# fferflo/semantic-meshes

Hardware: AMD Instinct MI355X
Metric: views/sec fused (1080p, 19 classes, 1M-tri mesh) (higher is better)
Workload: dtype f32; 1 GPU; cfg2: 1000000-triangle grid mesh, 11763 views/GPU at 1920x1080, 19 classes, probs resident in HBM; views_per_call=8, group_pipeline=True, repeats=1, allreduce=none, exchange=allreduce, nranks=1, allreduce_bytes=0, exchange_parts=1, held_views=0

## Files before the change

semantic_meshes_amd/_lib.py:

```python
import ctypes
import os
import threading

_HERE = os.path.dirname(os.path.abspath(__file__))
LIB_PATH = os.environ.get("SMESH_LIB_PATH") or os.path.join(_HERE, "csrc", "libsmesh_hip.so")

OK, ERR_INVALID, ERR_RUNTIME, ERR_NODEVICE = 0, 1, 2, 3
MEM_HOST, MEM_DEVICE = 0, 1
IDX_U32, IDX_I32, IDX_U64, IDX_I64 = 0, 1, 2, 3
AGG_KINDS = {"Sum": 0, "Summax": 1, "Mul": 2}
PROF_FUSE_SCATTER, PROF_FUSE_HIST, PROF_RASTER, PROF_FINALIZE, PROF_EXCHANGE = 0, 1, 2, 3, 4

c_void_p, c_int, c_u64, c_u32, c_float = ctypes.c_void_p, ctypes.c_int, ctypes.c_uint64, ctypes.c_uint32, ctypes.c_float
P = ctypes.POINTER


class CameraPOD(ctypes.Structure):
    _fields_ = [
        ("rotation", ctypes.c_float * 9),
        ("translation", ctypes.c_float * 3),
        ("focal", ctypes.c_double * 2),
        ("principal", ctypes.c_double * 2),
        ("width", ctypes.c_uint64),
        ("height", ctypes.c_uint64),
# ... 111 lines not shown
EVAL_SIGNATURES = {
    "smesh_confusion_create": (c_int, [c_u32, c_int, P(c_void_p)]),
    "smesh_confusion_destroy": (c_int, [c_void_p]),
    "smesh_confusion_reset": (c_int, [c_void_p]),
    "smesh_confusion_get": (c_int, [c_void_p, c_void_p, P(c_u64)]),
    "smesh_confusion_add_counts": (c_int, [c_void_p, c_void_p, c_u64]),
    "smesh_confusion_add_labels": (c_int, [c_void_p, c_void_p, c_int, c_void_p, c_int, c_int, c_u64]),
    "smesh_aggregator_labels": (c_int, [c_void_p, c_float, c_void_p, c_int]),
    "smesh_confusion_add_image": (c_int, [c_void_p, c_void_p, c_int, P(ctypes.c_int64), c_int, c_void_p, c_u64, c_int,
                                          c_void_p, c_int, P(ctypes.c_int64), c_int, c_u64, c_u64]),
    "smesh_confusion_add_view": (c_int, [c_void_p, c_void_p, P(CameraPOD), c_void_p, c_u64, c_void_p, c_int, P(ctypes.c_int64), c_int]),
    "smesh_confusion_add_views": (c_int, [c_void_p, c_void_p, P(CameraPOD), c_u64, c_void_p, c_u64, P(c_void_p), c_int,
                                          P(ctypes.c_int64), c_int]),
}

_lib = None
_lock = threading.Lock()


def _elf_dynamic_strings(path):
    import struct
    with open(path, "rb") as f:
        data = f.read()
    try:
        if data[:6] != b"\x7fELF\x02\x01":
            raise ValueError("not a little-endian ELF64 file")
        phoff, = struct.unpack_from("<Q", data, 0x20)
        phentsize, phnum = struct.unpack_from("<HH", data, 0x36)
        loads, dyn = [], None
        for k in range(phnum):
# ... 81 lines not shown
    if os.path.exists(rccl):
        os.environ.setdefault("SMESH_RCCL_LIB", rccl)


def lib():
    global _lib
    if _lib is None:
        with _lock:
            if _lib is None:
                if not os.path.exists(LIB_PATH):
                    raise RuntimeError(
                        "semantic_meshes_amd: %s not found -- build it with `make -C semantic_meshes_amd/csrc` "
                        "(or `python -c 'import __graft_entry__ as g; g.build()'`). There is no CPU fallback." % LIB_PATH)
                _preload_hip_runtime()
                L = ctypes.CDLL(LIB_PATH)
                for name, (res, args) in list(SIGNATURES.items()) + list(EXT_SIGNATURES.items()) + list(VERTEX_SIGNATURES.items()) + list(EVAL_SIGNATURES.items()):
                    fn = getattr(L, name)
                    fn.restype = res
                    fn.argtypes = args
                _lib = L
    return _lib


def check(status):
    if status == OK:
        return
    msg = lib().smesh_last_error().decode(errors="replace")
    if status == ERR_INVALID:
        raise ValueError(msg)
    raise RuntimeError(msg)

# ... 29 lines not shown
```

semantic_meshes_amd/csrc/common.hpp:

```cpp
#pragma once

#include <hip/hip_runtime.h>

#include <cstdint>
#include <cstdio>
#include <cstdlib>
#include <functional>
#include <mutex>
#include <string>
#include <vector>

#include "../../include/smesh.h"

namespace smesh {

int fail(int code, const std::string& msg);
int fail_hip(hipError_t e, const char* what, const char* file, int line);

#define SMESH_HIP(expr)                                                         \
  do {                                                                          \
    hipError_t _e = (expr);                                                     \
    if (_e != hipSuccess) return ::smesh::fail_hip(_e, #expr, __FILE__, __LINE__); \
  } while (0)

// ... 41 lines not shown
  bool counted = false;
  ProfScope(DeviceCtx* c, int s, hipStream_t stream = nullptr);
  ~ProfScope();
};

void prof_note(DeviceCtx* ctx, int slot, uint64_t launches, uint64_t views);

hipError_t dev_malloc(void** out, size_t bytes);
hipError_t dev_free(void* p, bool foreign = false);
uint64_t dev_cached_bytes(int device);
void dev_trim(int device);
void dev_cache_stats(uint64_t* live_blocks, uint64_t* cached_blocks, uint64_t* cached_bytes);

bool opt_group_pipeline();
bool opt_confusion_wave_aggregate();

constexpr uint32_t kConfusionLdsMaxC = 180;

struct Scratch {
  void* ptr = nullptr;
  size_t bytes = 0;
  int reserve(size_t need);
  void release();
};

inline uint64_t div_up(uint64_t a, uint64_t b) { return (a + b - 1) / b; }

inline int env_int(const char* name, int def) {
  const char* e = getenv(name);
  return e ? atoi(e) : def;
// ... 109 lines not shown
```

semantic_meshes_amd/csrc/context.cpp:

```cpp
#include "common.hpp"
#include "labels_scratch.hpp"

#include <algorithm>
#include <atomic>

#include <cstdlib>
#include <cstring>
#include <map>
#include <memory>
#include <unordered_map>
#include <vector>

namespace smesh {

static thread_local std::string g_err;

int fail(int code, const std::string& msg) {
  g_err = msg;
  return code;
}

int fail_hip(hipError_t e, const char* what, const char* file, int line) {
  char buf[512];
  snprintf(buf, sizeof buf, "HIP error %d (%s) at %s:%d: %s", (int)e, hipGetErrorString(e), file, line, what);
  g_err = buf;
  (void)hipGetLastError();
  return (e == hipErrorNoDevice || e == hipErrorInvalidDevice) ? SMESH_ERR_NODEVICE : SMESH_ERR_RUNTIME;
}

static std::atomic<int> g_confusion_wave_aggregate{1};
bool opt_confusion_wave_aggregate() { return g_confusion_wave_aggregate.load() != 0; }

static std::atomic<int> g_group_pipeline{-1};
bool opt_group_pipeline() {
  int v = g_group_pipeline.load();
  if (v < 0) {
    const char* e = getenv("SMESH_GROUP_PIPELINE");
    v = e ? (atoi(e) != 0 ? 1 : 0) : 1;
    g_group_pipeline.store(v);
  }
  return v != 0;
}

static std::mutex g_ctx_mu;
static std::vector<std::unique_ptr<DeviceCtx>> g_ctx;

// ... 233 lines not shown

using namespace smesh;

void smesh_last_fuse_instance(int* slot, int* views);

extern "C" {

const char* smesh_backend(void) { return "hip-gfx950"; }

const char* smesh_last_error(void) { return g_err.c_str(); }

int smesh_set_option(const char* name, int64_t value) {
  if (!name) return fail(SMESH_ERR_INVALID, "option name is NULL");
  if (!strcmp(name, "group_pipeline")) { g_group_pipeline.store(value != 0 ? 1 : 0); return SMESH_OK; }
  if (!strcmp(name, "confusion_wave_aggregate")) { g_confusion_wave_aggregate.store(value != 0 ? 1 : 0); return SMESH_OK; }
  return fail(SMESH_ERR_INVALID, std::string("unknown option: ") + name);
}
int smesh_get_option(const char* name, int64_t* value) {
  if (!name || !value) return fail(SMESH_ERR_INVALID, "NULL argument");
  if (!strcmp(name, "group_pipeline")) { *value = opt_group_pipeline() ? 1 : 0; return SMESH_OK; }
  if (!strcmp(name, "labels_lds_max_classes")) { *value = (int64_t)kLabelsLdsMaxC; return SMESH_OK; }
  if (!strcmp(name, "confusion_lds_max_classes")) { *value = (int64_t)kConfusionLdsMaxC; return SMESH_OK; }
  if (!strcmp(name, "confusion_wave_aggregate")) { *value = opt_confusion_wave_aggregate() ? 1 : 0; return SMESH_OK; }
  const bool want_slot = !strcmp(name, "last_fuse_slot");
  if (want_slot || !strcmp(name, "last_fuse_views")) {
    int slot, views;
    smesh_last_fuse_instance(&slot, &views);
    *value = want_slot ? slot : views;
    return SMESH_OK;
  }
  return fail(SMESH_ERR_INVALID, std::string("unknown option: ") + name);
}

int smesh_device_count(int* count) {
  if (!count) return fail(SMESH_ERR_INVALID, "count is NULL");
  int n = 0;
  if (hipGetDeviceCount(&n) != hipSuccess) {
    (void)hipGetLastError();
// ... 259 lines not shown
```

semantic_meshes_amd/csrc/raster.hip:

```cpp
#include "common.hpp"

#include <algorithm>
#include <cmath>
#include <cstdlib>
#include <cstring>
#include <new>
#include <string>
#include <utility>
#include <vector>

#pragma clang fp contract(off)

using namespace smesh;

struct smesh_aggregator;
int smesh_aggregator_add_device_contig(smesh_aggregator* a, const uint32_t* d_idx, const float* d_probs,
                                       const float* d_w, uint64_t W, uint64_t H);
bool smesh_aggregator_can_fuse_triangles(smesh_aggregator* a, uint64_t F);
bool smesh_aggregator_can_fuse_pair(smesh_aggregator* a);
int smesh_aggregator_max_fused_views(smesh_aggregator* a);
bool smesh_aggregator_takes_strided_probs(smesh_aggregator* a, int64_t ps0, int64_t ps1, int nviews);
int smesh_aggregator_dense_probs(smesh_aggregator* a, const float* d_probs, const int64_t ps[3], uint64_t W, uint64_t H, const float** out);
bool smesh_aggregator_fuses_small_views_by_mask(smesh_aggregator* a);
int smesh_aggregator_fuse_triangles(smesh_aggregator* a, uint64_t F, const uint32_t* prim_id, uint32_t big_capacity,
// ... 43 lines not shown
  s.u = 0.0; s.v = 0.0; s.iz = 0.0;
  const bool fin = isfinite(xc) && isfinite(yc) && isfinite(zc);
  if (zc > kNear && fin) {
    const double zd = (double)zc;
    const double u = cam.fx * ((double)xc / zd) + cam.cx;
    const double v = cam.fy * ((double)yc / zd) + cam.cy;
    if (isfinite(u) && isfinite(v)) {
      s.u = u; s.v = v; s.iz = 1.0 / zd;
    }
  } else if (fin) {
    s.iz = kBehind;
  }
  return s;
}

__device__ __forceinline__ void project_vertex(const float* __restrict__ verts, uint64_t V, const CameraArgs& cam,
                                               ScreenVertex* __restrict__ sv, uint32_t* __restrict__ big_count, const uint64_t i) {
  if (i == 0) { big_count[0] = 0u; big_count[1] = 0u; big_count[2] = 0u; big_count[3] = 0u; big_count[4] = 0u; big_count[5] = 0u; }
  if (i >= V) return;
  sv[i] = project_point(cam, verts[3 * i + 0], verts[3 * i + 1], verts[3 * i + 2]);
}

__global__ void k_project_vertices(const float* __restrict__ verts, uint64_t V, CameraArgs cam,
                                   ScreenVertex* __restrict__ sv, uint32_t* __restrict__ big_count) {
  project_vertex(verts, V, cam, sv, big_count, (uint64_t)blockIdx.x * blockDim.x + threadIdx.x);
}

constexpr int kMaxGroup = 8;
struct ProjectGroup {
  const float* verts;
  uint64_t V;
  CameraArgs cam[kMaxGroup];
  ScreenVertex* sv[kMaxGroup];
  uint32_t* big_count[kMaxGroup];
  uint32_t n;
};
__global__ void k_project_vertices_group(ProjectGroup g) {
  const uint64_t i = (uint64_t)blockIdx.x * blockDim.x + threadIdx.x;
  if (i == 0)
    for (uint32_t v = 0; v < g.n; v++)
      for (int k = 0; k < 6; k++) g.big_count[v][k] = 0u;
  if (i >= g.V) return;
  const float X = g.verts[3 * i + 0], Y = g.verts[3 * i + 1], Z = g.verts[3 * i + 2];
  for (uint32_t v = 0; v < g.n; v++) g.sv[v][i] = project_point(g.cam[v], X, Y, Z);
}

struct EdgeEq {
  double A, B, C;
};

__device__ __forceinline__ EdgeEq make_edge(double ax, double ay, double bx, double by) {
  EdgeEq e;
  const bool sw = (bx < ax) || (bx == ax && by < ay);
  const double lx = sw ? bx : ax, ly = sw ? by : ay;
  e.A = ay - by;
  e.B = bx - ax;
// ... 108 lines not shown
  uint64_t F, V;
  uint32_t W, H;
  uint32_t* big_queue;
  uint32_t* huge_queue;
  uint32_t* big_count;
  uint32_t big_capacity;
  TriFrag* frags;
  uint8_t* kinds;
  FragQueues q;
  uint32_t tpw;
  uint32_t groups;
  uint32_t* med_queue;
  uint32_t balance;
  uint32_t wg_push;
  uint32_t spread;
  uint32_t idx_optional;
};

__device__ __forceinline__ uint64_t key_index(uint32_t x, uint32_t y, uint32_t H) { return (uint64_t)x * H + y; }

__device__ __forceinline__ bool load_tri(const RasterArgs& a, uint64_t f, Tri& t, const int32_t i0, const int32_t i1, const int32_t i2);
__device__ __forceinline__ bool load_tri(const RasterArgs& a, uint64_t f, Tri& t) {
  return load_tri(a, f, t, a.faces[3 * f + 0], a.faces[3 * f + 1], a.faces[3 * f + 2]);
}
__device__ __forceinline__ bool load_tri(const RasterArgs& a, uint64_t f, Tri& t, const int32_t i0, const int32_t i1, const int32_t i2) {
  if ((uint64_t)max((uint32_t)i0, max((uint32_t)i1, (uint32_t)i2)) >= a.V) return false;
  if (a.tex_res && a.tex_res[f] == 0) return false;
  const ScreenVertex va = a.sv[i0], vb = a.sv[i1], vc = a.sv[i2];
  return setup_tri(va, vb, vc, a.W, a.H, t);
}
// ... 570 lines not shown
  for (uint32_t i = wave; i < turns; i += nwaves) {
    const int tri = lane / kLanes;
    const uint32_t e = i * (uint32_t)kTris + (uint32_t)tri;
    uint64_t fs = a.F;
    if (tri < kTris && e < nl) fs = a.med_queue[a.big_capacity - 1u - e];
    int32_t s0 = 0, s1 = 0, s2 = 0;
    if (fs < a.F) { s0 = a.faces[3 * fs + 0]; s1 = a.faces[3 * fs + 1]; s2 = a.faces[3 * fs + 2]; }
    raster_frag_64<TEX ? 6 : 2>(a, fs, s0, s1, s2, i & (kQSub - 1), lane % kLanes, true);
  }
}
template <bool TEX>
__global__ __launch_bounds__(256) void k_raster_medium(RasterArgs a) {
  raster_medium_wave<TEX>(a, (blockIdx.x * blockDim.x + threadIdx.x) >> 6, (gridDim.x * blockDim.x) >> 6);
}

template <bool LOOP, int MODE>
__device__ __forceinline__ void raster_frag_wave(const RasterArgs& a, const uint64_t wave_id) {
  const int lane = threadIdx.x & 63;
  if constexpr ((MODE & 2) != 0) {
    const int tri = lane / kSpread;
    uint64_t fs = wave_id * (uint64_t)kSpreadTris + (uint64_t)tri;
    if (tri >= kSpreadTris || fs >= a.F) fs = a.F;
    int32_t s0 = 0, s1 = 0, s2 = 0;
    if (fs < a.F) { s0 = a.faces[3 * fs + 0]; s1 = a.faces[3 * fs + 1]; s2 = a.faces[3 * fs + 2]; }
    raster_frag_64<MODE>(a, fs, s0, s1, s2, (uint32_t)wave_id & (kQSub - 1), lane % kSpread);
    return;
  } else {
  const uint32_t G = LOOP ? a.groups : 1u;
  uint64_t f = lane < (int)a.tpw ? wave_id * G * a.tpw + lane : a.F;
  int32_t n0 = 0, n1 = 0, n2 = 0;
  if (f < a.F) { n0 = a.faces[3 * f + 0]; n1 = a.faces[3 * f + 1]; n2 = a.faces[3 * f + 2]; }
  for (uint32_t g = 0; g < G; g++) {
    const int32_t i0 = n0, i1 = n1, i2 = n2;
    const uint64_t fn = f + 64u;
    if (g + 1 < G && fn < a.F) { n0 = a.faces[3 * fn + 0]; n1 = a.faces[3 * fn + 1]; n2 = a.faces[3 * fn + 2]; }
    raster_frag_64<MODE>(a, f, i0, i1, i2, (uint32_t)(wave_id * G + g) & (kQSub - 1));
    f = fn < a.F ? fn : a.F;
  }
  }
}

__device__ __forceinline__ uint32_t xcd_block(const uint32_t xcd, const uint32_t s, const uint32_t run) {
  const uint32_t q = s / run;
  return (q * 8u + xcd) * run + (s - q * run);
}
inline uint32_t xcd_slots(uint32_t nblocks, uint32_t run) { return (uint32_t)div_up(nblocks, 8u * run) * run; }

template <int MODE>
__global__ __launch_bounds__(256) __attribute__((amdgpu_waves_per_eu((MODE & 3) ? 4 : 5, 5))) void k_raster_frag(RasterArgs a, uint32_t nblocks, uint32_t chunk) {
  const uint32_t tb = chunk ? xcd_block(blockIdx.x & 7u, blockIdx.x >> 3, chunk) : blockIdx.x;
  if (tb >= nblocks) return;
  raster_frag_wave<false, MODE>(a, ((uint64_t)tb * blockDim.x + threadIdx.x) >> 6);
// ... 281 lines not shown

struct ImagePair {
  uint32_t* idx;
  float* depth;
  uint64_t pixels;
  bool idx_out, depth_out;
};

struct smesh_renderer {
  DeviceCtx* ctx = nullptr;
  uint64_t V = 0, F = 0, num_primitives = 0;
  float* verts = nullptr;
  int32_t* faces = nullptr;
  struct Bounds { bool valid = false; double lo[3] = {0, 0, 0}, hi[3] = {0, 0, 0}, max_edge = 0, mean_edge = 0; } bounds;
  uint32_t* prim_id = nullptr;
  struct ViewScratch {
    ScreenVertex* sv = nullptr;
    uint32_t* huge_queue = nullptr;
    uint32_t* med_queue = nullptr;
    unsigned long long* keys = nullptr;
    uint64_t keys_pixels = 0;
    FragQueues fq;
    uint64_t fq_tiles = 0;
  } vs[kSlots];
  bool texels = false;
  uint32_t* tex_res = nullptr;
  uint32_t* tex_first = nullptr;
  std::vector<int32_t> h_faces;
  std::vector<uint32_t> h_res, h_first;
  struct Side {
    uint32_t* big_queue = nullptr;
    uint32_t* big_count = nullptr;
    TriFrag* frags = nullptr;
    uint8_t* kinds = nullptr;
// ... 184 lines not shown
                       const smesh_camera_t* cam = nullptr) {
  RasterArgs a;
  a.faces = r->faces; a.verts = r->verts; a.sv = vs.sv; a.tex_res = r->texels ? r->tex_res : nullptr; a.tex_first = r->tex_first;
  a.prim_id = r->prim_id;
  a.keys = vs.keys; a.F = r->F; a.V = r->V; a.W = (uint32_t)W; a.H = (uint32_t)H;
  a.big_queue = r->side[side].big_queue; a.big_count = r->side[side].big_count; a.big_capacity = r->big_capacity;
  a.huge_queue = vs.huge_queue;
  a.med_queue = vs.med_queue;
  {
    static const int knob = env_int("SMESH_RASTER_BALANCE", -1);
    a.balance = (vs.med_queue && (knob >= 0 ? knob != 0 : (cam && depth_spread(r, cam) > 6.0))) ? (nviews > 1 ? 1u : 2u) : 0u;
  }
  a.frags = r->side[side].frags;
  a.kinds = r->side[side].kinds;
  a.q = FragQueues();
  a.idx_optional = 0u;
  a.tpw = 64;
  const bool fine = r->F >= 32768u;
  const uint64_t min_waves = fine ? 1024u : 2048u;
  const uint64_t launch_views = fine ? (uint64_t)std::max(1, nviews) : 1u;
  while (a.tpw > 1 && launch_views * r->F / a.tpw < min_waves) a.tpw >>= 1;
  a.groups = 1;
  a.spread = 0u;
  {
    static const int knob = env_int("SMESH_RASTER_WG_PUSH", -1);
    a.wg_push = knob >= 0 ? (uint32_t)(knob != 0) : (cam && typical_edge_pixels(r, cam) >= 5.0 ? 1u : 0u);
  }
  if (want_spread(r, cam, nviews)) { a.spread = (uint32_t)kSpread; a.tpw = (uint32_t)kSpreadTris; }
  return a;
}

uint32_t frag_groups(uint64_t F, int views, uint32_t tpw) {
  static const int knob = env_int("SMESH_RASTER_GROUPS", 0);
  if (tpw != 64u) return 1u;
  if (knob >= 1) return (uint32_t)knob;
  return (F >= 4000000u && (uint64_t)views * div_up(F, 256u) >= 20480u) ? 4u : 1u;
}

int render_into(smesh_renderer* r, const smesh_camera_t* cam, uint32_t* d_idx, float* d_depth, hipStream_t st = nullptr,
                int side = 0, int idx_optional = 0) {
  DeviceCtx* ctx = r->ctx;
  r->last_render_side = side;
  if (!st) {
    st = ctx->stream;
    SMESH_TRY(main_after_raster(r));
    r->main_pending = true;
  }
  const uint64_t W = cam->width, H = cam->height, N = W * H;
  smesh_renderer::ViewScratch& vs = r->vs[0];
  SMESH_TRY(ensure_keys(vs, W, H, st));
  ProfScope prof(ctx, SMESH_PROF_RASTER, st);
  const CameraArgs ca = camera_args(cam);
  RasterArgs a = raster_args(r, vs, side, W, H, 1, cam);
  a.cam = ca;
  if (r->V) {
    hipLaunchKernelGGL(k_project_vertices, dim3((uint32_t)div_up(r->V, 256)), dim3(256), 0, st, r->verts, r->V, ca, vs.sv,
                       r->side[side].big_count);
    SMESH_HIP(hipGetLastError());
  } else {
    SMESH_HIP(hipMemsetAsync(r->side[side].big_count, 0, 32, st));
  }
  if (r->F) {
    a.idx_optional = (idx_optional && plane_optional_allowed(r)) ? (uint32_t)idx_optional : 0u;
    const uint32_t big_grid = (uint32_t)std::min<uint64_t>(r->F, (uint64_t)ctx->num_cus);
    int qs = SMESH_OK;
    if (raster_path() == RasterPath::Frag && ensure_queues(r, vs, W, H, st, &qs)) {
      a.q = vs.fq;
      {
        const uint32_t nblocks = (uint32_t)div_up(div_up(r->F, a.tpw), 4);
        const uint32_t chunk = nblocks >= 64u ? kRasterXcdRun : 0u;
        const dim3 grid(chunk ? 8u * xcd_slots(nblocks, chunk) : nblocks);
        switch (raster_mode(a)) {
// ... 20 lines not shown
    }
    SMESH_TRY(qs);
    hipLaunchKernelGGL(k_raster_small, dim3((uint32_t)div_up(r->F, 256)), dim3(256), 0, st, a);
    SMESH_HIP(hipGetLastError());
    hipLaunchKernelGGL(k_raster_big, dim3(big_grid), dim3(256), 0, st, a, 0u);
    SMESH_HIP(hipGetLastError());
  }
  hipLaunchKernelGGL(k_resolve, dim3((uint32_t)div_up(N, 256)), dim3(256), 0, st, vs.keys, d_idx, d_depth, (uint32_t)W, (uint32_t)H);
  SMESH_HIP(hipGetLastError());
  SMESH_HIP(hipMemsetAsync(r->side[side].big_count + 1, 0xFF, 4, st));
  return SMESH_OK;
}

hipError_t alloc_side(smesh_renderer* r, int i);

hipError_t alloc_scratch(smesh_renderer* r, int i) {
  smesh_renderer::ViewScratch& vs = r->vs[i];
  hipError_t e = hipSuccess;
  if (!vs.sv) e = dev_malloc(reinterpret_cast<void**>(&vs.sv), std::max<uint64_t>(r->V * sizeof(ScreenVertex), 16));
  if (e == hipSuccess && !vs.huge_queue) e = dev_malloc(reinterpret_cast<void**>(&vs.huge_queue), (size_t)r->big_capacity * 4);
  if (e == hipSuccess && !vs.med_queue) e = dev_malloc(reinterpret_cast<void**>(&vs.med_queue), (size_t)r->big_capacity * 4);
  return e;
}

bool queues_fit_group(uint64_t W, uint64_t H) {
  if (raster_path() != RasterPath::Frag) return false;
  if (frag_cap_forced()) return true;
  const uint64_t ntiles = div_up(W, kQW) * div_up(H, kQH);
  const uint64_t cap = 16ull * kQPixels / kQSub;
  return ntiles * kQSub * cap * 10 <= (2ull << 30);
}

int prepare_group_slots(smesh_renderer* r, const smesh_camera_t* cams, int n, hipStream_t st, int base) {
  for (int v = 0; v < n; v++) {
    const uint64_t W = cams[v].width, H = cams[v].height, N = W * H;
    SMESH_HIP(alloc_side(r, base + v));
// ... 52 lines not shown
  rg.n = (uint32_t)n;
  {
    int votes = 0;
    for (int v = 0; v < n; v++) votes += want_spread(r, &cams[v], n) ? 1 : 0;
    if (2 * votes >= n && votes > 0)
      for (int v = 0; v < n; v++) { rg.view[v].spread = (uint32_t)kSpread; rg.view[v].tpw = (uint32_t)kSpreadTris; }
    int push_votes = 0;
    for (int v = 0; v < n; v++) push_votes += rg.view[v].wg_push ? 1 : 0;
    for (int v = 0; v < n; v++) rg.view[v].wg_push = 2 * push_votes >= n && push_votes > 0 ? 1u : 0u;
    int balance_votes = 0;
    for (int v = 0; v < n; v++) balance_votes += rg.view[v].balance ? 1 : 0;
    for (int v = 0; v < n; v++) rg.view[v].balance = 2 * balance_votes >= n && balance_votes > 0 ? (n > 1 ? 1u : 2u) : 0u;
  }
  for (int v = 0; v < n; v++) rg.view[v].groups = frag_groups(r->F, n, rg.view[0].tpw);
  rg.blocks_per_view = (uint32_t)div_up(div_up(r->F, rg.view[0].tpw * rg.view[0].groups), 4);
  ProfScope prof(ctx, SMESH_PROF_RASTER, st);
  hipLaunchKernelGGL(k_project_vertices_group, dim3((uint32_t)div_up(r->V, 256)), dim3(256), 0, st, pg);
  SMESH_HIP(hipGetLastError());
  {
    rg.chunk = rg.blocks_per_view >= 64u ? kRasterXcdRun : 0u;
    const dim3 grid(rg.chunk ? 8u * xcd_slots(rg.blocks_per_view, rg.chunk) * (uint32_t)n : (uint32_t)n * rg.blocks_per_view);
    switch (raster_mode(rg.view[0])) {
      case 7:  hipLaunchKernelGGL(k_raster_frag_group<7>, grid, dim3(256), 0, st, rg); break;
      case 5:  hipLaunchKernelGGL(k_raster_frag_group<5>, grid, dim3(256), 0, st, rg); break;
      case 4:  hipLaunchKernelGGL(k_raster_frag_group<4>, grid, dim3(256), 0, st, rg); break;
      case 3:  hipLaunchKernelGGL(k_raster_frag_group<3>, grid, dim3(256), 0, st, rg); break;
      case 1:  hipLaunchKernelGGL(k_raster_frag_group<1>, grid, dim3(256), 0, st, rg); break;
      default: hipLaunchKernelGGL(k_raster_frag_group<0>, grid, dim3(256), 0, st, rg); break;
    }
    if ((raster_mode(rg.view[0]) & 3) != 0 && rg.view[0].balance) {
      const uint32_t per_view = std::max(64u, 4u * (uint32_t)std::max(1, ctx->num_cus) / (uint32_t)n);
      if (rg.view[0].tex_res) hipLaunchKernelGGL(k_raster_medium_group<true>, dim3((uint32_t)n * per_view), dim3(256), 0, st, rg, per_view);
// ... 106 lines not shown
  const double eps = 32.0 * 5.9604644775390625e-08 * mag;
  const double z_lo = zmin - eps;
  const double L = std::sqrt(frob2) * b.max_edge + 4.0 * eps;
  if (!(z_lo > 1e-3) || !std::isfinite(mag) || !std::isfinite(L)) return INFINITY;
  const double ratio = L / z_lo;
  if (!(ratio < 0.25)) return INFINITY;
  const double fx = std::fabs(cam->focal[0]), fy = std::fabs(cam->focal[1]);
  const double ax = std::max(std::fabs(cam->principal[0]), std::fabs(W - cam->principal[0])) + 1.0;
  const double ay = std::max(std::fabs(cam->principal[1]), std::fabs(H - cam->principal[1])) + 1.0;
  const double du = (fx + ax) * ratio / (1.0 - ratio), dv = (fy + ay) * ratio / (1.0 - ratio);
  if (!std::isfinite(du) || !std::isfinite(dv)) return INFINITY;
  return std::max(du, dv);
}
bool no_huge_possible(const smesh_renderer* r, const smesh_camera_t* cam) { return box_extent_bound(r->bounds, cam) <= (double)kMedium - 4.0; }
bool no_big_possible(const smesh_renderer* r, const smesh_camera_t* cam) { return box_extent_bound(r->bounds, cam) <= 6.5; }

int create_common(const float* vertices, uint64_t V, const int32_t* faces, uint64_t F, int device,
                  smesh_renderer** out) {
  if (!out) return fail(SMESH_ERR_INVALID, "out is NULL");
  *out = nullptr;
  if ((V && !vertices) || (F && !faces)) return fail(SMESH_ERR_INVALID, "NULL mesh arrays");
  if (F >= 0xFFFFFFFFull || V >= 0x7FFFFFFFull) return fail(SMESH_ERR_INVALID, "mesh too large for 32-bit indices");
  DeviceCtx* ctx;
  SMESH_TRY(get_ctx(device, &ctx));
  SMESH_HIP(hipSetDevice(device));
  auto* r = new (std::nothrow) smesh_renderer();
  if (!r) return fail(SMESH_ERR_RUNTIME, "out of memory");
  r->ctx = ctx; r->V = V; r->F = F; r->num_primitives = F;
  r->big_capacity = (uint32_t)std::max<uint64_t>(F, 1);
  mesh_bounds(vertices, V, faces, F, r->bounds);
  hipError_t e = dev_malloc(reinterpret_cast<void**>(&r->verts), std::max<uint64_t>(V * 12, 16));
  if (e == hipSuccess) e = dev_malloc(reinterpret_cast<void**>(&r->faces), std::max<uint64_t>(F * 12, 16));
  if (e == hipSuccess) e = dev_malloc(reinterpret_cast<void**>(&r->vs[0].sv), std::max<uint64_t>(V * sizeof(ScreenVertex), 16));
  if (e == hipSuccess) e = alloc_side(r, 0);
  if (e == hipSuccess) e = dev_malloc(reinterpret_cast<void**>(&r->vs[0].huge_queue), (size_t)r->big_capacity * 4);
  if (e == hipSuccess) e = dev_malloc(reinterpret_cast<void**>(&r->vs[0].med_queue), (size_t)r->big_capacity * 4);
  if (e == hipSuccess && V) e = hipMemcpyAsync(r->verts, vertices, V * 12, hipMemcpyHostToDevice, ctx->stream);
  if (e == hipSuccess && F) e = hipMemcpyAsync(r->faces, faces, F * 12, hipMemcpyHostToDevice, ctx->stream);
  if (e == hipSuccess) e = hipStreamSynchronize(ctx->stream);
  if (e != hipSuccess) {
    smesh_renderer_destroy(r);
    return fail_hip(e, "renderer allocation/upload", __FILE__, __LINE__);
  }
  *out = r;
  return SMESH_OK;
}

}

static bool spatial_order(const float* v, uint64_t V, const int32_t* f, uint64_t F, std::vector<uint32_t>& order) {
  const char* env = getenv("SMESH_REORDER");
// ... 211 lines not shown
  hipError_t e = dev_malloc(reinterpret_cast<void**>(&r->tex_res), std::max<uint64_t>(F * 4, 16));
  if (e == hipSuccess) e = dev_malloc(reinterpret_cast<void**>(&r->tex_first), std::max<uint64_t>(F * 4, 16));
  if (e == hipSuccess && F) e = hipMemcpyAsync(r->tex_res, r->h_res.data(), F * 4, hipMemcpyHostToDevice, ctx->stream);
  if (e == hipSuccess && F) e = hipMemcpyAsync(r->tex_first, r->h_first.data(), F * 4, hipMemcpyHostToDevice, ctx->stream);
  if (e == hipSuccess) e = hipStreamSynchronize(ctx->stream);
  if (e != hipSuccess) { smesh_renderer_destroy(r); return fail_hip(e, "texel table upload", __FILE__, __LINE__); }
  *out = r;
  return SMESH_OK;
}

int smesh_renderer_destroy(smesh_renderer_t* r) {
  if (!r) return SMESH_OK;
  (void)hipSetDevice(r->ctx->device);
  (void)hipStreamSynchronize(r->ctx->raster_stream);
  (void)hipStreamSynchronize(r->ctx->stream);
  for (void* p : {(void*)r->prim_id, (void*)r->verts, (void*)r->faces, (void*)r->tex_res, (void*)r->tex_first})
    if (p) (void)dev_free(p);
  for (auto& sd : r->side)
    for (void* p : {(void*)sd.big_queue, (void*)sd.big_count, (void*)sd.frags, (void*)sd.kinds})
      if (p) (void)dev_free(p);
  for (auto& vs : r->vs)
    for (void* p : {(void*)vs.sv, (void*)vs.huge_queue, (void*)vs.med_queue, (void*)vs.keys, (void*)vs.fq.key, (void*)vs.fq.pix, (void*)vs.fq.count, (void*)vs.fq.flag})
      if (p) (void)dev_free(p);
  for (auto& im : r->images) { (void)dev_free(im.idx); (void)dev_free(im.depth); }
  r->own_idx.release();
  r->match_stage.release();
  if (r->d_hash) (void)dev_free(r->d_hash);
  for (int sd = 0; sd < kRecordSides; sd++)
    if (r->hash_ev[sd]) (void)hipEventDestroy(r->hash_ev[sd]);
  for (auto& f : r->fused) f.release();
  for (int i = 0; i < 2; i++) {
    if (i == 0 && r->ev_main_fence) (void)hipEventDestroy(r->ev_main_fence);
    if (r->ev_bank_rendered[i]) (void)hipEventDestroy(r->ev_bank_rendered[i]);
    if (r->ev_bank_consumed[i]) (void)hipEventDestroy(r->ev_bank_consumed[i]);
  }
  delete r;
  return SMESH_OK;
// ... 523 lines not shown
  for (int sd = 0; sd < kRecordSides; sd++) {
    if (r->last_idx[sd] != indices_dev || !r->rec_valid[sd] || r->hash_valid[sd]) continue;
    SMESH_HIP(hipSetDevice(ctx->device));
    if (!r->d_hash) {
      SMESH_HIP(dev_malloc(reinterpret_cast<void**>(&r->d_hash), (kRecordSides + 1) * sizeof(unsigned long long)));
      SMESH_HIP(hipMemsetAsync(r->d_hash, 0, (kRecordSides + 1) * sizeof(unsigned long long), ctx->stream));
    }
    SMESH_TRY(plane_checksum(ctx, ctx->stream, indices_dev, r->last_W[sd] * r->last_H[sd], r->d_hash + sd));
    if (!r->hash_ev[sd]) SMESH_HIP(hipEventCreateWithFlags(&r->hash_ev[sd], hipEventDisableTiming));
    SMESH_HIP(hipEventRecord(r->hash_ev[sd], ctx->stream));
    r->hash_valid[sd] = true;
  }
  return SMESH_OK;
}

int smesh_box_extent_bound(const float* vertices, uint64_t V, const int32_t* faces, uint64_t F, const smesh_camera_t* cam, double* bound) {
  if (!cam || !bound || (V && !vertices) || (F && !faces)) return fail(SMESH_ERR_INVALID, "NULL argument");
  smesh_renderer::Bounds b;
  mesh_bounds(vertices, V, faces, F, b);
  *bound = box_extent_bound(b, cam);
  return SMESH_OK;
}

int smesh_renderer_render_stats(smesh_renderer_t* r, const smesh_camera_t* cam, int* huge_stage_needed, uint32_t queue_lengths[4]) {
  if (!r || !cam) return fail(SMESH_ERR_INVALID, "NULL argument");
  SMESH_TRY(check_camera(cam));
  std::lock_guard<std::mutex> g(r->mu);
  if (huge_stage_needed) *huge_stage_needed = (no_huge_possible(r, cam) ? 0 : 1) | (no_big_possible(r, cam) ? 0 : 2);
  if (queue_lengths) {
    DeviceCtx* ctx = r->ctx;
// ... 11 lines not shown
```

semantic_meshes_amd/render.py:

```python
import ctypes

import numpy as np

from . import _lib
from .data import Camera
from .device import DeviceArray


def _mesh_arrays(mesh):
    v = np.ascontiguousarray(getattr(mesh, "vertices"), dtype=np.float32)
    f = np.ascontiguousarray(getattr(mesh, "faces"), dtype=np.int32)
    if v.ndim != 2 or v.shape[1] != 3 or f.ndim != 2 or f.shape[1] != 3:
        raise ValueError("mesh must provide vertices[V,3] and faces[F,3]")
    return v, f


import os
import weakref

RETURN_CAPSULES = os.environ.get("SMESH_RENDER_CAPSULES", "0") == "1"

_live_renderers = weakref.WeakSet()

LAZY_RENDER = os.environ.get("SMESH_LAZY_RENDER", "1") != "0"
# ... 132 lines not shown
        self._lazy_unrun = False
        if capsules:
            return indices.capsule(), depth.capsule()
        return indices, depth

    def render_stats(self, camera, queues=True):
        if queues and self._lazy_unrun:
            _lib.flush_pending(self.device)
            self.render(camera, capsules=False, lazy=False)
        needed = ctypes.c_int()
        q = (ctypes.c_uint32 * 4)()
        _lib.check(_lib.lib().smesh_renderer_render_stats(self._h, ctypes.byref(camera._pod), ctypes.byref(needed),
                                                         ctypes.cast(q, ctypes.c_void_p) if queues else None))
        self.last_big_stage_needed = bool(needed.value & 2)
        return bool(needed.value & 1), [int(x) for x in q]

    def render_numpy(self, camera):
        W, H = camera.resolution
        idx = np.empty((W, H), np.uint32)
        depth = np.empty((W, H), np.float32)
        _lib.check(_lib.lib().smesh_renderer_render(self._h, ctypes.byref(camera._pod),
                                                   idx.ctypes.data_as(ctypes.c_void_p), depth.ctypes.data_as(ctypes.c_void_p)))
        return idx, depth

    def _face_rows(self, source, threshold, normalize, on_device):
        from .fusion import _MeshAggregator, _dense_rows
        from .device import DeviceBuffer, release_to, result_empty
        if not getattr(self, "is_texel", False):
            raise ValueError("face_annotations needs a texel renderer (render.texels): the primitives of this one are its faces")
        P, F = self.getPrimitivesNum(), self._num_faces
# ... 71 lines not shown
```

Baseline: 16420 views/s.

## Cull 64-triangle runs against the view frustum before fragment rasterization

Precomputes an axis-aligned bounding box for every run of 64 consecutive faces at mesh creation. During vertex projection it tests each box conservatively against the camera frustum and near plane, writing a per-run visibility byte. The fragment raster wave then skips face loads and rasterization for invisible runs, writing empty fragment records instead. This adds per-view box tests and a visibility buffer, and only helps when runs of spatially coherent faces fall fully outside the view.

```diff
diff --git a/include/smesh_raster.h b/include/smesh_raster.h
--- /dev/null
+++ b/include/smesh_raster.h
@@ -0,0 +1,16 @@
+#ifndef SMESH_RASTER_H
+#define SMESH_RASTER_H
+
+#include "smesh.h"
+
+#ifdef __cplusplus
+extern "C" {
+#endif
+
+int smesh_renderer_cull_stats(smesh_renderer_t* r, uint64_t* runs, uint32_t skipped[8], int* views);
+
+#ifdef __cplusplus
+}
+#endif
+
+#endif
diff --git a/semantic_meshes_amd/_lib.py b/semantic_meshes_amd/_lib.py
--- a/semantic_meshes_amd/_lib.py
+++ b/semantic_meshes_amd/_lib.py
@@ -149,6 +149,10 @@
                                           P(ctypes.c_int64), c_int]),
 }
 
+RASTER_SIGNATURES = {
+    "smesh_renderer_cull_stats": (c_int, [c_void_p, P(c_u64), c_void_p, P(c_int)]),
+}
+
 _lib = None
 _lock = threading.Lock()
 
@@ -260,7 +264,7 @@
                         "(or `python -c 'import __graft_entry__ as g; g.build()'`). There is no CPU fallback." % LIB_PATH)
                 _preload_hip_runtime()
                 L = ctypes.CDLL(LIB_PATH)
-                for name, (res, args) in list(SIGNATURES.items()) + list(EXT_SIGNATURES.items()) + list(VERTEX_SIGNATURES.items()) + list(EVAL_SIGNATURES.items()):
+                for name, (res, args) in list(SIGNATURES.items()) + list(EXT_SIGNATURES.items()) + list(VERTEX_SIGNATURES.items()) + list(EVAL_SIGNATURES.items()) + list(RASTER_SIGNATURES.items()):
                     fn = getattr(L, name)
                     fn.restype = res
                     fn.argtypes = args
diff --git a/semantic_meshes_amd/csrc/common.hpp b/semantic_meshes_amd/csrc/common.hpp
--- a/semantic_meshes_amd/csrc/common.hpp
+++ b/semantic_meshes_amd/csrc/common.hpp
@@ -79,6 +79,7 @@
 
 bool opt_group_pipeline();
 bool opt_confusion_wave_aggregate();
+bool opt_raster_cull();
 
 constexpr uint32_t kConfusionLdsMaxC = 180;
 
diff --git a/semantic_meshes_amd/csrc/context.cpp b/semantic_meshes_amd/csrc/context.cpp
--- a/semantic_meshes_amd/csrc/context.cpp
+++ b/semantic_meshes_amd/csrc/context.cpp
@@ -30,6 +30,9 @@
 
 static std::atomic<int> g_confusion_wave_aggregate{1};
 bool opt_confusion_wave_aggregate() { return g_confusion_wave_aggregate.load() != 0; }
+
+static std::atomic<int> g_raster_cull{1};
+bool opt_raster_cull() { return g_raster_cull.load() != 0; }
 
 static std::atomic<int> g_group_pipeline{-1};
 bool opt_group_pipeline() {
@@ -293,6 +296,7 @@
   if (!name) return fail(SMESH_ERR_INVALID, "option name is NULL");
   if (!strcmp(name, "group_pipeline")) { g_group_pipeline.store(value != 0 ? 1 : 0); return SMESH_OK; }
   if (!strcmp(name, "confusion_wave_aggregate")) { g_confusion_wave_aggregate.store(value != 0 ? 1 : 0); return SMESH_OK; }
+  if (!strcmp(name, "raster_cull")) { g_raster_cull.store(value != 0 ? 1 : 0); return SMESH_OK; }
   return fail(SMESH_ERR_INVALID, std::string("unknown option: ") + name);
 }
 int smesh_get_option(const char* name, int64_t* value) {
@@ -301,6 +305,7 @@
   if (!strcmp(name, "labels_lds_max_classes")) { *value = (int64_t)kLabelsLdsMaxC; return SMESH_OK; }
   if (!strcmp(name, "confusion_lds_max_classes")) { *value = (int64_t)kConfusionLdsMaxC; return SMESH_OK; }
   if (!strcmp(name, "confusion_wave_aggregate")) { *value = opt_confusion_wave_aggregate() ? 1 : 0; return SMESH_OK; }
+  if (!strcmp(name, "raster_cull")) { *value = opt_raster_cull() ? 1 : 0; return SMESH_OK; }
   const bool want_slot = !strcmp(name, "last_fuse_slot");
   if (want_slot || !strcmp(name, "last_fuse_views")) {
     int slot, views;
diff --git a/semantic_meshes_amd/csrc/raster.hip b/semantic_meshes_amd/csrc/raster.hip
--- a/semantic_meshes_amd/csrc/raster.hip
+++ b/semantic_meshes_amd/csrc/raster.hip
@@ -1,4 +1,5 @@
 #include "common.hpp"
+#include "../../include/smesh_raster.h"
 
 #include <algorithm>
 #include <cmath>
@@ -81,16 +82,50 @@
   return s;
 }
 
+constexpr uint32_t kRun = 64;
+__device__ __forceinline__ bool run_invisible(const CameraArgs& cam, const float* __restrict__ box) {
+  const double lo[3] = {(double)box[0], (double)box[1], (double)box[2]}, hi[3] = {(double)box[3], (double)box[4], (double)box[5]};
+  if (!(lo[0] <= hi[0])) return false;
+  double m[3], err[3];
+  for (int r = 0; r < 3; r++) {
+    m[r] = fabs((double)cam.t[r]);
+    for (int d = 0; d < 3; d++) m[r] += fabs((double)cam.R[3 * r + d]) * fmax(fabs(lo[d]), fabs(hi[d]));
+    err[r] = 8.0 * 5.9604644775390625e-08 * m[r] + 1e-30;
+  }
+  if (!isfinite(m[0]) || !isfinite(m[1]) || !isfinite(m[2])) return false;
+  const double W = (double)cam.W, H = (double)cam.H;
+  const double cl = cam.cx + 1.0, cr = cam.cx - W - 1.0, ct = cam.cy + 1.0, cb = cam.cy - H - 1.0;
+  const double el = fabs(cam.fx) * err[0] + fabs(cl) * err[2], er = fabs(cam.fx) * err[0] + fabs(cr) * err[2];
+  const double et = fabs(cam.fy) * err[1] + fabs(ct) * err[2], eb = fabs(cam.fy) * err[1] + fabs(cb) * err[2];
+  const double zb = (double)kNear - err[2];
+  bool left = true, right = true, top = true, bottom = true, behind = true;
+  for (int c = 0; c < 8; c++) {
+    const double X = (c & 1) ? hi[0] : lo[0], Y = (c & 2) ? hi[1] : lo[1], Z = (c & 4) ? hi[2] : lo[2];
+    const double xc = (((double)cam.R[0] * X + (double)cam.R[1] * Y) + (double)cam.R[2] * Z) + (double)cam.t[0];
+    const double yc = (((double)cam.R[3] * X + (double)cam.R[4] * Y) + (double)cam.R[5] * Z) + (double)cam.t[1];
+    const double zc = (((double)cam.R[6] * X + (double)cam.R[7] * Y) + (double)cam.R[8] * Z) + (double)cam.t[2];
+    left = left && (cam.fx * xc + cl * zc <= -el);
+    right = right && (cam.fx * xc + cr * zc >= er);
+    top = top && (cam.fy * yc + ct * zc <= -et);
+    bottom = bottom && (cam.fy * yc + cb * zc >= eb);
+    behind = behind && (zc <= zb);
+  }
+  return left || right || top || bottom || behind;
+}
+
 __device__ __forceinline__ void project_vertex(const float* __restrict__ verts, uint64_t V, const CameraArgs& cam,
                                                ScreenVertex* __restrict__ sv, uint32_t* __restrict__ big_count, const uint64_t i) {
-  if (i == 0) { big_count[0] = 0u; big_count[1] = 0u; big_count[2] = 0u; big_count[3] = 0u; big_count[4] = 0u; big_count[5] = 0u; }
+  if (i == 0) { big_count[0] = 0u; big_count[1] = 0u; big_count[2] = 0u; big_count[3] = 0u; big_count[4] = 0u; big_count[5] = 0u; big_count[6] = 0u; }
   if (i >= V) return;
   sv[i] = project_point(cam, verts[3 * i + 0], verts[3 * i + 1], verts[3 * i + 2]);
 }
 
 __global__ void k_project_vertices(const float* __restrict__ verts, uint64_t V, CameraArgs cam,
-                                   ScreenVertex* __restrict__ sv, uint32_t* __restrict__ big_count) {
-  project_vertex(verts, V, cam, sv, big_count, (uint64_t)blockIdx.x * blockDim.x + threadIdx.x);
+                                   ScreenVertex* __restrict__ sv, uint32_t* __restrict__ big_count,
+                                   const float* __restrict__ run_boxes, uint32_t runs, uint8_t* __restrict__ vis) {
+  const uint64_t i = (uint64_t)blockIdx.x * blockDim.x + threadIdx.x;
+  if (run_boxes && i < runs) vis[i] = run_invisible(cam, run_boxes + 6 * i) ? 0 : 1;
+  project_vertex(verts, V, cam, sv, big_count, i);
 }
 
 constexpr int kMaxGroup = 8;
@@ -101,12 +136,17 @@
   ScreenVertex* sv[kMaxGroup];
   uint32_t* big_count[kMaxGroup];
   uint32_t n;
+  const float* run_boxes;
+  uint32_t runs;
+  uint8_t* vis[kMaxGroup];
 };
 __global__ void k_project_vertices_group(ProjectGroup g) {
   const uint64_t i = (uint64_t)blockIdx.x * blockDim.x + threadIdx.x;
   if (i == 0)
     for (uint32_t v = 0; v < g.n; v++)
-      for (int k = 0; k < 6; k++) g.big_count[v][k] = 0u;
+      for (int k = 0; k < 7; k++) g.big_count[v][k] = 0u;
+  if (g.run_boxes && i < g.runs)
+    for (uint32_t v = 0; v < g.n; v++) g.vis[v][i] = run_invisible(g.cam[v], g.run_boxes + 6 * i) ? 0 : 1;
   if (i >= g.V) return;
   const float X = g.verts[3 * i + 0], Y = g.verts[3 * i + 1], Z = g.verts[3 * i + 2];
   for (uint32_t v = 0; v < g.n; v++) g.sv[v][i] = project_point(g.cam[v], X, Y, Z);
@@ -245,6 +285,7 @@
   uint32_t balance;
   uint32_t wg_push;
   uint32_t spread;
+  const uint8_t* vis;
   uint32_t idx_optional;
 };
 
@@ -845,6 +886,13 @@
   raster_medium_wave<TEX>(a, (blockIdx.x * blockDim.x + threadIdx.x) >> 6, (gridDim.x * blockDim.x) >> 6);
 }
 
+__device__ __forceinline__ bool run_visible(const RasterArgs& a, const uint64_t fb) {
+  if (!a.vis || fb >= a.F) return true;
+  const uint32_t run = (uint32_t)(fb / kRun);
+  const uint32_t word = reinterpret_cast<const uint32_t*>(a.vis)[run >> 2];
+  return ((word >> (8u * (run & 3u))) & 0xFFu) != 0u;
+}
+
 template <bool LOOP, int MODE>
 __device__ __forceinline__ void raster_frag_wave(const RasterArgs& a, const uint64_t wave_id) {
   const int lane = threadIdx.x & 63;
@@ -857,16 +905,32 @@
     raster_frag_64<MODE>(a, fs, s0, s1, s2, (uint32_t)wave_id & (kQSub - 1), lane % kSpread);
     return;
   } else {
+  constexpr bool kCull = (MODE & 3) == 0;
   const uint32_t G = LOOP ? a.groups : 1u;
-  uint64_t f = lane < (int)a.tpw ? wave_id * G * a.tpw + lane : a.F;
+  uint64_t fb = ((uint64_t)(uint32_t)__builtin_amdgcn_readfirstlane((int)(uint32_t)(wave_id >> 32)) << 32 |
+                 (uint64_t)(uint32_t)__builtin_amdgcn_readfirstlane((int)(uint32_t)wave_id)) * G * a.tpw;
+  uint64_t f = lane < (int)a.tpw ? fb + lane : a.F;
+  bool vis_cur = !kCull || run_visible(a, fb);
   int32_t n0 = 0, n1 = 0, n2 = 0;
-  if (f < a.F) { n0 = a.faces[3 * f + 0]; n1 = a.faces[3 * f + 1]; n2 = a.faces[3 * f + 2]; }
+  if (vis_cur && f < a.F) { n0 = a.faces[3 * f + 0]; n1 = a.faces[3 * f + 1]; n2 = a.faces[3 * f + 2]; }
   for (uint32_t g = 0; g < G; g++) {
-    const int32_t i0 = n0, i1 = n1, i2 = n2;
     const uint64_t fn = f + 64u;
-    if (g + 1 < G && fn < a.F) { n0 = a.faces[3 * fn + 0]; n1 = a.faces[3 * fn + 1]; n2 = a.faces[3 * fn + 2]; }
-    raster_frag_64<MODE>(a, f, i0, i1, i2, (uint32_t)(wave_id * G + g) & (kQSub - 1));
+    const bool vis_next = g + 1 < G && (!kCull || run_visible(a, fb + 64u));
+    if (kCull && !vis_cur) {
+      if (f < a.F) {
+        if (a.frags && !a.kinds) { TriFrag rec; rec.x0 = 0; rec.y0 = 0; rec.kind = 0; rec.pad = 0; rec.mask = 0ull; a.frags[f] = rec; }
+        if (a.kinds) a.kinds[f] = (uint8_t)0;
+      }
+      if (lane == 0 && (fb & (uint64_t)(kRun - 1u)) == 0u) atomicAdd(a.big_count + 6, 1u);
+      if (vis_next && fn < a.F) { n0 = a.faces[3 * fn + 0]; n1 = a.faces[3 * fn + 1]; n2 = a.faces[3 * fn + 2]; }
+    } else {
+      const int32_t i0 = n0, i1 = n1, i2 = n2;
+      if (vis_next && fn < a.F) { n0 = a.faces[3 * fn + 0]; n1 = a.faces[3 * fn + 1]; n2 = a.faces[3 * fn + 2]; }
+      raster_frag_64<MODE>(a, f, i0, i1, i2, (uint32_t)(wave_id * G + g) & (kQSub - 1));
+    }
     f = fn < a.F ? fn : a.F;
+    fb += 64u;
+    vis_cur = vis_next;
   }
   }
 }
@@ -1178,10 +1242,14 @@
   int32_t* faces = nullptr;
   struct Bounds { bool valid = false; double lo[3] = {0, 0, 0}, hi[3] = {0, 0, 0}, max_edge = 0, mean_edge = 0; } bounds;
   uint32_t* prim_id = nullptr;
+  float* run_boxes = nullptr;
+  uint32_t runs = 0;
+  int cull_side = 0, cull_views = 0;
   struct ViewScratch {
     ScreenVertex* sv = nullptr;
     uint32_t* huge_queue = nullptr;
     uint32_t* med_queue = nullptr;
+    uint8_t* vis = nullptr;
     unsigned long long* keys = nullptr;
     uint64_t keys_pixels = 0;
     FragQueues fq;
@@ -1396,6 +1464,7 @@
   a.frags = r->side[side].frags;
   a.kinds = r->side[side].kinds;
   a.q = FragQueues();
+  a.vis = nullptr;
   a.idx_optional = 0u;
   a.tpw = 64;
   const bool fine = r->F >= 32768u;
@@ -1419,6 +1488,10 @@
   return (F >= 4000000u && (uint64_t)views * div_up(F, 256u) >= 20480u) ? 4u : 1u;
 }
 
+bool cull_this_launch(const smesh_renderer* r, const smesh_renderer::ViewScratch& vs, int mode) {
+  return opt_raster_cull() && r->run_boxes && vs.vis && r->V && (mode & 3) == 0;
+}
+
 int render_into(smesh_renderer* r, const smesh_camera_t* cam, uint32_t* d_idx, float* d_depth, hipStream_t st = nullptr,
                 int side = 0, int idx_optional = 0) {
   DeviceCtx* ctx = r->ctx;
@@ -1435,9 +1508,12 @@
   const CameraArgs ca = camera_args(cam);
   RasterArgs a = raster_args(r, vs, side, W, H, 1, cam);
   a.cam = ca;
+  r->cull_side = side; r->cull_views = 1;
   if (r->V) {
-    hipLaunchKernelGGL(k_project_vertices, dim3((uint32_t)div_up(r->V, 256)), dim3(256), 0, st, r->verts, r->V, ca, vs.sv,
-                       r->side[side].big_count);
+    const bool cull = raster_path() == RasterPath::Frag && cull_this_launch(r, vs, raster_mode(a));
+    if (cull) a.vis = vs.vis;
+    hipLaunchKernelGGL(k_project_vertices, dim3((uint32_t)div_up(std::max<uint64_t>(r->V, cull ? r->runs : 0u), 256)), dim3(256), 0, st,
+                       r->verts, r->V, ca, vs.sv, r->side[side].big_count, cull ? r->run_boxes : nullptr, r->runs, vs.vis);
     SMESH_HIP(hipGetLastError());
   } else {
     SMESH_HIP(hipMemsetAsync(r->side[side].big_count, 0, 32, st));
@@ -1488,12 +1564,15 @@
 
 hipError_t alloc_side(smesh_renderer* r, int i);
 
+inline size_t vis_bytes(uint32_t runs) { return std::max<size_t>(((size_t)runs + 3u) & ~(size_t)3u, 16); }
+
 hipError_t alloc_scratch(smesh_renderer* r, int i) {
   smesh_renderer::ViewScratch& vs = r->vs[i];
   hipError_t e = hipSuccess;
   if (!vs.sv) e = dev_malloc(reinterpret_cast<void**>(&vs.sv), std::max<uint64_t>(r->V * sizeof(ScreenVertex), 16));
   if (e == hipSuccess && !vs.huge_queue) e = dev_malloc(reinterpret_cast<void**>(&vs.huge_queue), (size_t)r->big_capacity * 4);
   if (e == hipSuccess && !vs.med_queue) e = dev_malloc(reinterpret_cast<void**>(&vs.med_queue), (size_t)r->big_capacity * 4);
+  if (e == hipSuccess && !vs.vis && r->run_boxes) e = dev_malloc(reinterpret_cast<void**>(&vs.vis), vis_bytes(r->runs));
   return e;
 }
 
@@ -1576,8 +1655,15 @@
   }
   for (int v = 0; v < n; v++) rg.view[v].groups = frag_groups(r->F, n, rg.view[0].tpw);
   rg.blocks_per_view = (uint32_t)div_up(div_up(r->F, rg.view[0].tpw * rg.view[0].groups), 4);
+  r->cull_side = side_base; r->cull_views = n;
+  bool cull = true;
+  for (int v = 0; v < n; v++) cull = cull && cull_this_launch(r, r->vs[base + v], raster_mode(rg.view[0]));
+  if (cull) {
+    pg.run_boxes = r->run_boxes; pg.runs = r->runs;
+    for (int v = 0; v < n; v++) { pg.vis[v] = r->vs[base + v].vis; rg.view[v].vis = r->vs[base + v].vis; }
+  }
   ProfScope prof(ctx, SMESH_PROF_RASTER, st);
-  hipLaunchKernelGGL(k_project_vertices_group, dim3((uint32_t)div_up(r->V, 256)), dim3(256), 0, st, pg);
+  hipLaunchKernelGGL(k_project_vertices_group, dim3((uint32_t)div_up(std::max<uint64_t>(r->V, cull ? r->runs : 0u), 256)), dim3(256), 0, st, pg);
   SMESH_HIP(hipGetLastError());
   {
     rg.chunk = rg.blocks_per_view >= 64u ? kRasterXcdRun : 0u;
@@ -1714,6 +1800,28 @@
 }
 bool no_huge_possible(const smesh_renderer* r, const smesh_camera_t* cam) { return box_extent_bound(r->bounds, cam) <= (double)kMedium - 4.0; }
 bool no_big_possible(const smesh_renderer* r, const smesh_camera_t* cam) { return box_extent_bound(r->bounds, cam) <= 6.5; }
+
+void build_run_boxes(const float* v, uint64_t V, const int32_t* f, uint64_t F, std::vector<float>& out) {
+  const uint64_t runs = div_up(F, kRun);
+  out.resize(6 * runs);
+  for (uint64_t k = 0; k < runs; k++) {
+    float lo[3] = {INFINITY, INFINITY, INFINITY}, hi[3] = {-INFINITY, -INFINITY, -INFINITY};
+    bool ok = true;
+    for (uint64_t i = k * kRun; i < std::min<uint64_t>(F, (k + 1) * kRun) && ok; i++)
+      for (int c = 0; c < 3 && ok; c++) {
+        const int32_t j = f[3 * i + c];
+        if (j < 0 || (uint64_t)j >= V) { ok = false; break; }
+        for (int d = 0; d < 3; d++) {
+          const float x = v[3 * (uint64_t)j + d];
+          ok = ok && std::isfinite(x);
+          lo[d] = std::min(lo[d], x); hi[d] = std::max(hi[d], x);
+        }
+      }
+    float* b = &out[6 * k];
+    if (ok) { for (int d = 0; d < 3; d++) { b[d] = lo[d]; b[3 + d] = hi[d]; } }
+    else    { for (int d = 0; d < 3; d++) { b[d] = 1.0f; b[3 + d] = -1.0f; } }
+  }
+}
 
 int create_common(const float* vertices, uint64_t V, const int32_t* faces, uint64_t F, int device,
                   smesh_renderer** out) {
@@ -1735,6 +1843,14 @@
   if (e == hipSuccess) e = alloc_side(r, 0);
   if (e == hipSuccess) e = dev_malloc(reinterpret_cast<void**>(&r->vs[0].huge_queue), (size_t)r->big_capacity * 4);
   if (e == hipSuccess) e = dev_malloc(reinterpret_cast<void**>(&r->vs[0].med_queue), (size_t)r->big_capacity * 4);
+  std::vector<float> boxes;
+  if (V && F) {
+    build_run_boxes(vertices, V, faces, F, boxes);
+    r->runs = (uint32_t)(boxes.size() / 6);
+    if (e == hipSuccess) e = dev_malloc(reinterpret_cast<void**>(&r->run_boxes), boxes.size() * 4);
+    if (e == hipSuccess) e = dev_malloc(reinterpret_cast<void**>(&r->vs[0].vis), vis_bytes(r->runs));
+    if (e == hipSuccess) e = hipMemcpyAsync(r->run_boxes, boxes.data(), boxes.size() * 4, hipMemcpyHostToDevice, ctx->stream);
+  }
   if (e == hipSuccess && V) e = hipMemcpyAsync(r->verts, vertices, V * 12, hipMemcpyHostToDevice, ctx->stream);
   if (e == hipSuccess && F) e = hipMemcpyAsync(r->faces, faces, F * 12, hipMemcpyHostToDevice, ctx->stream);
   if (e == hipSuccess) e = hipStreamSynchronize(ctx->stream);
@@ -1976,13 +2092,13 @@
   (void)hipSetDevice(r->ctx->device);
   (void)hipStreamSynchronize(r->ctx->raster_stream);
   (void)hipStreamSynchronize(r->ctx->stream);
-  for (void* p : {(void*)r->prim_id, (void*)r->verts, (void*)r->faces, (void*)r->tex_res, (void*)r->tex_first})
+  for (void* p : {(void*)r->prim_id, (void*)r->verts, (void*)r->faces, (void*)r->tex_res, (void*)r->tex_first, (void*)r->run_boxes})
     if (p) (void)dev_free(p);
   for (auto& sd : r->side)
     for (void* p : {(void*)sd.big_queue, (void*)sd.big_count, (void*)sd.frags, (void*)sd.kinds})
       if (p) (void)dev_free(p);
   for (auto& vs : r->vs)
-    for (void* p : {(void*)vs.sv, (void*)vs.huge_queue, (void*)vs.med_queue, (void*)vs.keys, (void*)vs.fq.key, (void*)vs.fq.pix, (void*)vs.fq.count, (void*)vs.fq.flag})
+    for (void* p : {(void*)vs.sv, (void*)vs.huge_queue, (void*)vs.med_queue, (void*)vs.vis, (void*)vs.keys, (void*)vs.fq.key, (void*)vs.fq.pix, (void*)vs.fq.count, (void*)vs.fq.flag})
       if (p) (void)dev_free(p);
   for (auto& im : r->images) { (void)dev_free(im.idx); (void)dev_free(im.depth); }
   r->own_idx.release();
@@ -2536,6 +2652,26 @@
   return SMESH_OK;
 }
 
+int smesh_renderer_cull_stats(smesh_renderer_t* r, uint64_t* runs, uint32_t skipped[8], int* views) {
+  if (!r) return fail(SMESH_ERR_INVALID, "NULL argument");
+  std::lock_guard<std::mutex> g(r->mu);
+  if (runs) *runs = r->runs;
+  if (views) *views = r->cull_views;
+  if (skipped) {
+    DeviceCtx* ctx = r->ctx;
+    std::lock_guard<std::recursive_mutex> lock(ctx->mu);
+    SMESH_HIP(hipSetDevice(ctx->device));
+    SMESH_HIP(hipStreamSynchronize(ctx->raster_stream));
+    for (int v = 0; v < kMaxGroup; v++) {
+      skipped[v] = 0u;
+      if (v < r->cull_views && r->side[r->cull_side + v].big_count)
+        SMESH_HIP(hipMemcpyAsync(skipped + v, r->side[r->cull_side + v].big_count + 6, 4, hipMemcpyDeviceToHost, ctx->stream));
+    }
+    SMESH_HIP(hipStreamSynchronize(ctx->stream));
+  }
+  return SMESH_OK;
+}
+
 int smesh_box_extent_bound(const float* vertices, uint64_t V, const int32_t* faces, uint64_t F, const smesh_camera_t* cam, double* bound) {
   if (!cam || !bound || (V && !vertices) || (F && !faces)) return fail(SMESH_ERR_INVALID, "NULL argument");
   smesh_renderer::Bounds b;
diff --git a/semantic_meshes_amd/render.py b/semantic_meshes_amd/render.py
--- a/semantic_meshes_amd/render.py
+++ b/semantic_meshes_amd/render.py
@@ -170,6 +170,14 @@
                                                          ctypes.cast(q, ctypes.c_void_p) if queues else None))
         self.last_big_stage_needed = bool(needed.value & 2)
         return bool(needed.value & 1), [int(x) for x in q]
+
+    def cull_stats(self):
+        _lib.flush_pending(self.device)
+        runs, views = ctypes.c_uint64(), ctypes.c_int()
+        skipped = (ctypes.c_uint32 * 8)()
+        _lib.check(_lib.lib().smesh_renderer_cull_stats(self._h, ctypes.byref(runs), ctypes.cast(skipped, ctypes.c_void_p),
+                                                       ctypes.byref(views)))
+        return int(runs.value), [int(skipped[v]) for v in range(views.value)]
 
     def render_numpy(self, camera):
         W, H = camera.resolution
```

New measurement: 15960 views/s. -2.8%, worse.
